# MoseleyBioinformaticsLab/pdb_eda

Measured on NVIDIA B200. Metric: voxels/s (atom-sphere voxels + blob-CCL voxels per pass of the voxel hot path), higher is better.
Workload: dtype f64

## Files before the change

### include/pdbeda_b200.h

```cpp
#ifndef PDBEDA_B200_H
#define PDBEDA_B200_H

#include <stdint.h>

#ifdef __cplusplus
extern "C" {
#endif

#define PE_ABI_VERSION 1

typedef enum pe_status {
    PE_OK = 0,
    PE_ERR_ARG = -1,
    PE_ERR_CUDA = -2,
    PE_ERR_CAPACITY = -3,
    PE_ERR_NO_DEVICE = -4
} pe_status;

typedef struct pe_geom {
    int32_t ncrs[3];
    int32_t crs_start[3];
    int32_t xyz_interval[3];
    int32_t crs_interval[3];
    int32_t unique_ncrs[3];
    int32_t map2xyz[3];
    int32_t map2crs[3];
    int32_t orthogonal;
    int32_t mv_perm[3];
    int32_t mv_fma;
    double grid_length[3];
    double origin[3];
    double ortho[9];
    double deortho[9];
} pe_geom;

int pe_abi_version(void);
const char *pe_last_error(void);
int pe_device_info(int32_t *sm_count, int32_t *cc_major, int32_t *cc_minor);

long long pe_launch_count(void);
void pe_profile_enable(int on);
void pe_profile_reset(void);
int pe_profile_entries(void);
int pe_profile_get(int index, const char **name, long long *count, double *total_ms);

int64_t pe_stats_workspace_bytes(void);
int pe_map_mean_std(const float *d_rho, int64_t n, double *d_out, void *d_ws, void *stream);
int pe_map_sum_abs(const float *d_rho, int64_t n, float cutoff, double *d_out, void *d_ws, void *stream);
int pe_sum_abs_f64(const double *d_values, int64_t n, float cutoff, double *d_out, void *d_ws, void *stream);

int pe_point_density(const pe_geom *g, const float *d_rho, int64_t n, const int32_t *d_crs, float *d_rho_out,
                     uint8_t *d_valid, void *stream);
int pe_xyz2crs(const pe_geom *g, int64_t n, const double *d_xyz, int32_t *d_crs, void *stream);
int pe_crs2xyz(const pe_geom *g, int64_t n, const int32_t *d_crs, double *d_xyz, void *stream);

#define PE_SPHERE_NOUT 8
int64_t pe_sphere_workspace_bytes(int64_t n_atoms);
int pe_sphere_union_warp_cycles(unsigned long long *out5);
int pe_sphere_sums(const pe_geom *g, const float *d_rho, int32_t n_atoms, const double *d_xyz,
                   const float *d_radius, int32_t n_groups, const int32_t *d_group_start, float cut_pos,
                   float cut_neg, double *d_out, void *d_ws, void *stream);
int pe_sphere_sums_atoms_and_groups(const pe_geom *g, const float *d_rho, int32_t n_atoms, const double *d_xyz,
                                    const float *d_atom_radius, float max_atom_radius, const float *d_group_radius,
                                    int32_t n_groups, const int32_t *d_group_start, float cut_pos, float cut_neg,
                                    double *d_out_atoms, double *d_out_groups, void *d_ws, void *stream);

typedef struct pe_sums_map {
    pe_geom geom;
    const float *d_rho;
    float cut_pos;
    float cut_neg;
} pe_sums_map;
int64_t pe_batch_sphere_sums_workspace_bytes(int64_t n_atoms);
int pe_batch_sphere_sums(int32_t n_maps, const pe_sums_map *d_maps, int32_t n_atoms, const double *d_xyz, const float *d_radius,
                         int32_t n_groups, const int32_t *d_group_map, const int32_t *d_group_start, const int32_t *d_atom_start,
                         double *d_out, void *d_ws, void *stream);

int pe_sphere_count(const pe_geom *g, const float *d_rho, int32_t n_atoms, const double *d_xyz,
                    const float *d_radius, float cutoff, int32_t *d_count, int32_t *d_box, void *stream);
int pe_sphere_fill(const pe_geom *g, const float *d_rho, int32_t n_atoms, const double *d_xyz,
                   const float *d_radius, float cutoff, const int64_t *d_offset, int32_t max_box_voxels,
                   int32_t *d_index, float *d_value, int32_t *d_label, void *stream);

int64_t pe_blob_workspace_bytes(const pe_geom *g, int64_t cap_voxels);
int pe_blob_stage_times(unsigned long long *out12);
int pe_blob_label(const pe_geom *g, const float *d_rho, float cut_pos, float cut_neg, int64_t cap_voxels,
                  int64_t cap_blobs, int64_t *d_counts, uint32_t *d_key, float *d_value, int32_t *d_label,
                  double *d_stats, void *d_ws, void *stream);

int64_t pe_slab_exchange_bytes(int64_t cap_blobs, int64_t cap_plane);
int64_t pe_slab_workspace_bytes(int32_t world, int64_t cap_blobs, int32_t u0, int32_t u1);
int pe_slab_boundary(const pe_geom *g_slab, int32_t u2_whole, int32_t s0, int32_t last_is_cut, const int64_t *d_counts,
                     int64_t cap_voxels, const uint32_t *d_key, const int32_t *d_label, int64_t cap_blobs, int64_t cap_plane,
                     void *d_exchange, void *d_ws, void *stream);
int pe_slab_merge(int32_t world, int32_t rank, const void *d_gathered, int64_t cap_blobs, int64_t cap_plane, int32_t u0,
                  int32_t u1, int32_t *d_new_number, int64_t *d_n_merged, void *d_ws, void *stream);
int pe_slab_relabel(const pe_geom *g_whole, int32_t u2_slab, int32_t s0, const int64_t *d_counts, int64_t cap_voxels,
                    const uint32_t *d_key, const float *d_value, int32_t *d_label, int64_t cap_blobs,
                    const int32_t *d_new_number, const int64_t *d_n_merged, int64_t cap_merged, double *d_stats, void *d_ws,
                    void *stream);
int pe_slab_status(const void *d_ws, void *stream, int32_t *bad);

int64_t pe_cluster_workspace_bytes(int64_t n);
int pe_cluster_crs(int64_t n, const int32_t *d_crs, int32_t *d_label, int64_t *d_nclusters, void *d_ws,
                   void *stream);
int pe_cluster_crs_grouped(int64_t n, const int32_t *d_crs, const int32_t *d_group, int32_t *d_label,
                           uint8_t *d_first, int64_t *d_nclusters, void *d_ws, void *stream);

int pe_crs_stats(const pe_geom *g, const float *d_rho, int64_t n, const int32_t *d_crs, const int32_t *d_label,
                 const uint8_t *d_take, int64_t n_clusters, double *d_stats, void *stream);

int pe_pair_metrics(const pe_geom *g, const float *d_rho_fo, const float *d_rho_diff, int64_t n, const int32_t *d_crs,
                    const int32_t *d_label, const uint8_t *d_take, int64_t n_groups, double *d_out, void *stream);

typedef struct pe_pair_map {
    pe_geom geom;
    const float *d_fo;
    const float *d_diff;
} pe_pair_map;
int64_t pe_pair_union_workspace_bytes(int32_t n_atoms);
int pe_pair_union_metrics(int32_t n_maps, const pe_pair_map *d_maps, int32_t n_groups, const int32_t *d_group_map,
                          const int32_t *d_group_start, const double *d_xyz, const float *d_radius, double *d_out, void *d_ws,
                          void *stream);

int64_t pe_overlap_workspace_bytes(int64_t n, int64_t cap_pairs);
int pe_overlap_pairs(int64_t n, const int32_t *d_crs, const int32_t *d_owner, const int32_t *d_group,
                     int64_t cap_pairs, int64_t *d_npairs, int32_t *d_pairs, void *d_ws, void *stream);
// ... 38 lines not shown
```

### pdb_eda_b200/_lib.py

```python
import ctypes
import os

_HERE = os.path.dirname(os.path.abspath(__file__))
LIB_PATH = os.path.join(_HERE, "csrc", "libpdbeda_b200.so")

PE_SPHERE_NOUT = 8


class PeGeom(ctypes.Structure):
    _fields_ = [
        ("ncrs", ctypes.c_int32 * 3),
        ("crs_start", ctypes.c_int32 * 3),
        ("xyz_interval", ctypes.c_int32 * 3),
        ("crs_interval", ctypes.c_int32 * 3),
        ("unique_ncrs", ctypes.c_int32 * 3),
        ("map2xyz", ctypes.c_int32 * 3),
        ("map2crs", ctypes.c_int32 * 3),
        ("orthogonal", ctypes.c_int32),
        ("mv_perm", ctypes.c_int32 * 3),
        ("mv_fma", ctypes.c_int32),
        ("grid_length", ctypes.c_double * 3),
        ("origin", ctypes.c_double * 3),
        ("ortho", ctypes.c_double * 9),
        ("deortho", ctypes.c_double * 9),
    ]


class PeBatchMap(ctypes.Structure):
    _fields_ = [("geom", PeGeom), ("d_rho", ctypes.c_void_p), ("cutoff", ctypes.c_float), ("atom_begin", ctypes.c_int32),
                ("atom_end", ctypes.c_int32), ("reserved", ctypes.c_int32)]


class PeSumsMap(ctypes.Structure):
    _fields_ = [("geom", PeGeom), ("d_rho", ctypes.c_void_p), ("cut_pos", ctypes.c_float), ("cut_neg", ctypes.c_float)]


class PePairMap(ctypes.Structure):
    _fields_ = [("geom", PeGeom), ("d_fo", ctypes.c_void_p), ("d_diff", ctypes.c_void_p)]


class PdbEdaLibError(RuntimeError):
    pass


_P = ctypes.c_void_p
_I32 = ctypes.c_int32
_I64 = ctypes.c_int64
_F32 = ctypes.c_float
_GEOM = ctypes.POINTER(PeGeom)

SIGNATURES = {
    "pe_abi_version": (ctypes.c_int, []),
    "pe_last_error": (ctypes.c_char_p, []),
    "pe_device_info": (ctypes.c_int, [ctypes.POINTER(_I32)] * 3),
    "pe_launch_count": (ctypes.c_longlong, []),
    "pe_profile_enable": (None, [ctypes.c_int]),
    "pe_profile_reset": (None, []),
    "pe_profile_entries": (ctypes.c_int, []),
    "pe_profile_get": (ctypes.c_int, [ctypes.c_int, ctypes.POINTER(ctypes.c_char_p), ctypes.POINTER(ctypes.c_longlong),
                                      ctypes.POINTER(ctypes.c_double)]),
    "pe_stats_workspace_bytes": (_I64, []),
    "pe_map_mean_std": (ctypes.c_int, [_P, _I64, _P, _P, _P]),
    "pe_map_sum_abs": (ctypes.c_int, [_P, _I64, _F32, _P, _P, _P]),
    "pe_sum_abs_f64": (ctypes.c_int, [_P, _I64, _F32, _P, _P, _P]),
    "pe_point_density": (ctypes.c_int, [_GEOM, _P, _I64, _P, _P, _P, _P]),
    "pe_xyz2crs": (ctypes.c_int, [_GEOM, _I64, _P, _P, _P]),
    "pe_crs2xyz": (ctypes.c_int, [_GEOM, _I64, _P, _P, _P]),
    "pe_sphere_workspace_bytes": (_I64, [_I64]),
    "pe_sphere_union_warp_cycles": (ctypes.c_int, [ctypes.POINTER(ctypes.c_ulonglong)]),
    "pe_sphere_sums": (ctypes.c_int, [_GEOM, _P, _I32, _P, _P, _I32, _P, _F32, _F32, _P, _P, _P]),
    "pe_sphere_sums_atoms_and_groups": (ctypes.c_int, [_GEOM, _P, _I32, _P, _P, _F32, _P, _I32, _P, _F32, _F32, _P, _P, _P, _P]),
    "pe_sphere_count": (ctypes.c_int, [_GEOM, _P, _I32, _P, _P, _F32, _P, _P, _P]),
    "pe_sphere_fill": (ctypes.c_int, [_GEOM, _P, _I32, _P, _P, _F32, _P, _I32, _P, _P, _P, _P]),
    "pe_blob_workspace_bytes": (_I64, [_GEOM, _I64]),
    "pe_blob_stage_times": (ctypes.c_int, [ctypes.POINTER(ctypes.c_ulonglong)]),
    "pe_blob_label": (ctypes.c_int, [_GEOM, _P, _F32, _F32, _I64, _I64, _P, _P, _P, _P, _P, _P, _P]),
    "pe_cluster_workspace_bytes": (_I64, [_I64]),
    "pe_cluster_crs": (ctypes.c_int, [_I64, _P, _P, _P, _P, _P]),
    "pe_cluster_crs_grouped": (ctypes.c_int, [_I64, _P, _P, _P, _P, _P, _P, _P]),
    "pe_crs_stats": (ctypes.c_int, [_GEOM, _P, _I64, _P, _P, _P, _I64, _P, _P]),
    "pe_pair_metrics": (ctypes.c_int, [_GEOM, _P, _P, _I64, _P, _P, _P, _I64, _P, _P]),
    "pe_batch_sphere_sums_workspace_bytes": (_I64, [_I64]),
    "pe_batch_sphere_sums": (ctypes.c_int, [_I32, _P, _I32, _P, _P, _I32, _P, _P, _P, _P, _P, _P]),
    "pe_pair_union_workspace_bytes": (_I64, [_I32]),
    "pe_pair_union_metrics": (ctypes.c_int, [_I32, _P, _I32, _P, _P, _P, _P, _P, _P, _P]),
    "pe_overlap_workspace_bytes": (_I64, [_I64, _I64]),
    "pe_overlap_pairs": (ctypes.c_int, [_I64, _P, _P, _P, _I64, _P, _P, _P, _P]),
    "pe_symmetry_workspace_bytes": (_I64, [_I32, _I32]),
    "pe_symmetry_expand": (ctypes.c_int, [_GEOM, _I32, _P, _I32, _P, _P, ctypes.POINTER(ctypes.c_double),
                                          ctypes.POINTER(ctypes.c_double), _I64, _P, _P, _P, _P, _P, _P]),
    "pe_nearest_atom": (ctypes.c_int, [_I64, _P, _I64, _P, _P, _P, _P]),
    "pe_slab_exchange_bytes": (_I64, [_I64, _I64]),
    "pe_slab_workspace_bytes": (_I64, [_I32, _I64, _I32, _I32]),
    "pe_slab_boundary": (ctypes.c_int, [_GEOM, _I32, _I32, _I32, _P, _I64, _P, _P, _I64, _I64, _P, _P, _P]),
    "pe_slab_merge": (ctypes.c_int, [_I32, _I32, _P, _I64, _I64, _I32, _I32, _P, _P, _P, _P]),
    "pe_slab_relabel": (ctypes.c_int, [_GEOM, _I32, _I32, _P, _I64, _P, _P, _P, _I64, _P, _P, _I64, _P, _P, _P]),
    "pe_slab_status": (ctypes.c_int, [_P, _P, ctypes.POINTER(_I32)]),
    "pe_cloud_workspace_bytes": (_I64, [_I64, _I64, _I64, _I64]),
    "pe_cloud_count": (ctypes.c_int, [_I32, _P, _I32, _P, _P, _P, _P, _P, _P, _P, _P]),
    "pe_cloud_aggregate": (ctypes.c_int, [_I32, _P, _I32, _P, _P, _P, _P, _P, _P, _P, _I32, _P, _I64, _I32, ctypes.c_double, _P, _P, _P,
                                          _P, _P]),
    "pe_cloud_status": (ctypes.c_int, [_P, _P, ctypes.POINTER(_I32)]),
    "pe_cloud_statistics": (ctypes.c_int, [_I32, _P, _I32, _P, _P, _P, _P, _I32, _P, _P, _P, _P, _I32, _P, _P, ctypes.c_double, _P, _P,
                                           _P, _P]),
}

_lib = None


def load():
    global _lib
    if _lib is not None:
        return _lib
    if not os.path.isfile(LIB_PATH):
        raise PdbEdaLibError(
            "%s not found: build it with `python -c 'import __graft_entry__ as g; g.build()'` or "
            "`make -C pdb_eda_b200/csrc` (there is no CPU fallback)" % LIB_PATH)
    lib = ctypes.CDLL(LIB_PATH)
    for name, (restype, argtypes) in SIGNATURES.items():
        fn = getattr(lib, name)
        fn.restype = restype
        fn.argtypes = argtypes
    if lib.pe_abi_version() != 1:
        raise PdbEdaLibError("libpdbeda_b200.so ABI version %d, expected 1" % lib.pe_abi_version())
    _lib = lib
    return lib


def check(rc, what):
    if rc != 0:
        msg = load().pe_last_error()
        raise PdbEdaLibError("%s failed (%d): %s" % (what, rc, msg.decode("utf-8", "replace") if msg else "?"))


def require_device():
    lib = load()
    sm, major, minor = _I32(0), _I32(0), _I32(0)
    check(lib.pe_device_info(ctypes.byref(sm), ctypes.byref(major), ctypes.byref(minor)), "pe_device_info")
    return sm.value, major.value, minor.value


def profile(enable=None, reset=False):
    lib = load()
# ... 16 lines not shown
```

### pdb_eda_b200/csrc/pe_blob.cu

```cuda
#include <cooperative_groups.h>
#include "pe_common.cuh"

namespace cg = cooperative_groups;

namespace pe {

constexpr int kBmpTx = 32;
constexpr int kBmpTy = 8;
constexpr int kSparseThreads = 512;
constexpr int kSegShift = 9;
constexpr int kSegWords = 1 << kSegShift;
constexpr int kChunkShift = 9;
constexpr int kChunkSmem = 4096;
constexpr int kScanBlocksPerSm = 2;
constexpr int kQueueCap = 160;
constexpr int kPoolWords = (kSparseThreads / 32) * 3 * kQueueCap > kChunkSmem ? (kSparseThreads / 32) * 3 * kQueueCap : kChunkSmem;
static_assert((1 << kChunkShift) == kSparseThreads, "a ranking chunk is one block of voxels");

struct BlobPlan {
    int U0, U1, U2, W;
    int64_t nwords;
    int64_t nwords_pad;
    int64_t nseg;
    int64_t cap;
// ... 573 lines not shown
}

}

using namespace pe;

extern "C" {

int pe_blob_stage_times(unsigned long long *out12) {
    PE_CHECK_ARG(out12 != nullptr, "pe_blob_stage_times: null pointer");
    PE_CUDA(cudaMemcpyFromSymbol(out12, g_stage_ns, sizeof(unsigned long long) * 12));
    return PE_OK;
}

int64_t pe_blob_workspace_bytes(const pe_geom *g, int64_t cap_voxels) {
    if (!g || cap_voxels < 0) return -1;
    return make_plan(g, cap_voxels).total;
}

int pe_blob_label(const pe_geom *g, const float *d_rho, float cut_pos, float cut_neg, int64_t cap_voxels,
                  int64_t cap_blobs, int64_t *d_counts, uint32_t *d_key, float *d_value, int32_t *d_label,
                  double *d_stats, void *d_ws, void *stream) {
    if (int rc = check_geom(g)) return rc;
    PE_CHECK_ARG(d_rho && d_counts && d_key && d_value && d_label && d_stats && d_ws, "pe_blob_label: null pointer");
    PE_CHECK_ARG(cap_voxels > 0 && cap_blobs > 0, "pe_blob_label: capacities must be positive");
    PE_CHECK_ARG(cap_voxels < (1ll << 30), "pe_blob_label: cap_voxels must be below 2^30");
    PE_CHECK_ARG(!(cut_pos < 0.f) && !(cut_neg > 0.f), "pe_blob_label: cut_pos must be >= 0 and cut_neg <= 0");
    PE_CHECK_ARG(cut_pos == cut_pos && cut_neg == cut_neg, "pe_blob_label: NaN cutoff");
    const BlobPlan p = make_plan(g, cap_voxels);
    PE_CHECK_ARG((int64_t)p.U0 * p.U1 * p.U2 < (1ll << 32), "pe_blob_label: unique volume too large for 32-bit keys");
    PE_CHECK_ARG(p.nwords_pad < (1ll << 31), "pe_blob_label: bit planes too large");
    cudaStream_t st = (cudaStream_t)stream;
    char *ws = (char *)d_ws;
    const int NC = g->ncrs[0], NR = g->ncrs[1];
    uint32_t *bmp = (uint32_t *)(ws + p.off_bmp);
    const bool use_pos = cut_pos > 0.f, use_neg = cut_neg < 0.f;

    PE_CUDA(cudaMemsetAsync(d_counts, 0, 5 * sizeof(int64_t), st));
    uint32_t *segcount = (uint32_t *)(ws + p.off_seg);
    PE_CUDA(cudaMemsetAsync(segcount, 0, (size_t)align_up(p.nseg * 4, 256) + 1024, st));
    {
        const bool vec4 = (NC % 4 == 0) && (((uintptr_t)d_rho & 15u) == 0);
        const int vec = vec4 ? 4 : 1;
        const int tx = kBmpTx, ty = kBmpTy;
        dim3 block(tx, ty, 1);
        dim3 grid(p.W / kWordsPerThread, (p.U0 + tx * vec - 1) / (tx * vec), (p.U1 + ty - 1) / ty);
        PE_CHECK_ARG(grid.y <= 65535 && grid.z <= 65535, "pe_blob_label: map too large for the launch grid");
        if (vec4)
            PE_LAUNCH("threshold_bitmap_kernel", st, threshold_bitmap_kernel<4><<<grid, block, 0, st>>>(
                d_rho, NC, NR, p.U0, p.U1, p.U2, p.W, cut_pos, cut_neg, use_pos, use_neg, bmp, bmp + p.nwords_pad, p.nwords_pad, segcount));
        else
            PE_LAUNCH("threshold_bitmap_kernel", st, threshold_bitmap_kernel<1><<<grid, block, 0, st>>>(
                d_rho, NC, NR, p.U0, p.U1, p.U2, p.W, cut_pos, cut_neg, use_pos, use_neg, bmp, bmp + p.nwords_pad, p.nwords_pad, segcount));
        PE_LAUNCH_CHECK();
    }
    SparseArgs a;
    a.rho = d_rho;
    a.NC = NC;
    a.NR = NR;
    a.U1 = p.U1;
    a.U2 = p.U2;
    a.W = p.W;
    a.nwords_pad = p.nwords_pad;
    a.cap = p.cap;
    a.cap_blobs = cap_blobs;
    a.nseg = (int)p.nseg;
    a.bmp = bmp;
    a.segcount = segcount;
    a.base = (uint32_t *)(ws + p.off_base);
    a.parent = (uint32_t *)(ws + p.off_parent);
    a.flags = (uint2 *)(ws + p.off_flags);
    a.coarse = (uint32_t *)(ws + p.off_coarse);
    a.nchunk_cap = p.nchunk_cap;
    a.counts = d_counts;
    a.key = d_key;
    a.value = d_value;
    a.label = d_label;
    a.stats = d_stats;
    static int blocks_per_sm = 0;
    if (blocks_per_sm == 0) {
        PE_CUDA(cudaOccupancyMaxActiveBlocksPerMultiprocessor(&blocks_per_sm, blob_sparse_kernel, kSparseThreads, 0));
        PE_CHECK_ARG(blocks_per_sm > 0, "pe_blob_label: the sparse kernel does not fit an SM");
    }
    const int nblocks = sm_count() * (blocks_per_sm < 3 ? blocks_per_sm : 3);
    a.p1_per_sm = blocks_per_sm == 3 ? kScanBlocksPerSm : (blocks_per_sm < 3 ? blocks_per_sm : 3);
    a.p1_blocks = sm_count() * a.p1_per_sm;
    a.sm_rank = (int *)(ws + p.off_seg + align_up(p.nseg * 4, 256));
    pe_geom geom = *g;
    void *args[] = {(void *)&geom, (void *)&a};
    PE_LAUNCH("blob_sparse_kernel", st,
              PE_CUDA(cudaLaunchCooperativeKernel((const void *)blob_sparse_kernel, dim3(nblocks), dim3(kSparseThreads), args, 0, st)));
    PE_LAUNCH_CHECK();
    return PE_OK;
}

}
```

### pdb_eda_b200/csrc/pe_common.cuh

```cuda
#pragma once
#include <cuda_runtime.h>
#include <stdint.h>
#include <stdio.h>
#include "../../include/pdbeda_b200.h"

namespace pe {

void set_error(const char *fmt, ...);

#define PE_CHECK_ARG(cond, ...)          \
    do {                                 \
        if (!(cond)) {                   \
            pe::set_error(__VA_ARGS__);  \
            return PE_ERR_ARG;           \
        }                                \
    } while (0)

#define PE_CUDA(call)                                                                         \
    do {                                                                                      \
        cudaError_t err__ = (call);                                                           \
        if (err__ != cudaSuccess) {                                                           \
            pe::set_error("%s failed at %s:%d: %s", #call, __FILE__, __LINE__,                \
                          cudaGetErrorString(err__));                                         \
            return PE_ERR_CUDA;                                                               \
        }                                                                                     \
    } while (0)

#define PE_LAUNCH_CHECK()                                                                     \
    do {                                                                                      \
        cudaError_t err__ = cudaGetLastError();                                               \
        if (err__ != cudaSuccess) {                                                           \
            pe::set_error("kernel launch failed at %s:%d: %s", __FILE__, __LINE__,            \
                          cudaGetErrorString(err__));                                         \
            return PE_ERR_CUDA;                                                               \
        }                                                                                     \
    } while (0)

struct ProfScope {
    int slot;
    cudaStream_t stream;
    ProfScope(const char *tag, cudaStream_t st);
    ~ProfScope();
};
#define PE_LAUNCH(tag, stream, ...)                          \
    do {                                                     \
        pe::ProfScope prof_scope__(tag, (cudaStream_t)(stream)); \
        __VA_ARGS__;                                         \
    } while (0)

int sm_count();
int check_geom(const pe_geom *g);
int check_geom_shape(const pe_geom *g, int64_t *nvox_out);

static inline int64_t align_up(int64_t x, int64_t a) { return (x + a - 1) / a * a; }

constexpr int kWarp = 32;
constexpr unsigned kFull = 0xffffffffu;
constexpr int kInvalidOff = (int)0x80000000;

__device__ __forceinline__ int sel3(int a0, int a1, int a2, int i) { return i == 0 ? a0 : (i == 1 ? a1 : a2); }
__device__ __forceinline__ double sel3(double a0, double a1, double a2, int i) { return i == 0 ? a0 : (i == 1 ? a1 : a2); }

__device__ __forceinline__ int floordiv(int a, int b) {
    int q = a / b;
    if ((a % b != 0) && ((a < 0) != (b < 0))) --q;
    return q;
}

__device__ __forceinline__ int wrap_index(int k, int n, int interval) {
    if (k < 0 || k >= n) k -= floordiv(k, interval) * interval;
    if ((n <= k && k < interval) || k < 0) return -1;
    return k;
}

__device__ __forceinline__ double mv_row(const double *a, double x0, double x1, double x2, const pe_geom &g) {
    const int p0 = g.mv_perm[0], p1 = g.mv_perm[1], p2 = g.mv_perm[2];
    const double a0 = a[p0], a1 = a[p1], a2 = a[p2];
    const double y0 = sel3(x0, x1, x2, p0), y1 = sel3(x0, x1, x2, p1), y2 = sel3(x0, x1, x2, p2);
    double acc = __dmul_rn(a0, y0);
    if (g.mv_fma) {
        acc = __fma_rn(a1, y1, acc);
        acc = __fma_rn(a2, y2, acc);
    } else {
        acc = __dadd_rn(acc, __dmul_rn(a1, y1));
        acc = __dadd_rn(acc, __dmul_rn(a2, y2));
    }
    return acc;
}

__device__ __forceinline__ int round_quotient(double a, double b) {
    const double q = __dmul_rn(a, __drcp_rn(b));
    const double r = rint(q);
    const double d = fabs(__dsub_rn(q, r));
    if (d < 0.499999999 && fabs(q) < 1.0e6) return (int)r;
    return (int)rint(__ddiv_rn(a, b));
}

__device__ __forceinline__ void xyz2crs(const pe_geom &g, double x, double y, double z, int &c, int &r, int &s) {
    int p0, p1, p2;
    if (g.orthogonal) {
        p0 = round_quotient(__dsub_rn(x, g.origin[0]), g.grid_length[0]);
        p1 = round_quotient(__dsub_rn(y, g.origin[1]), g.grid_length[1]);
        p2 = round_quotient(__dsub_rn(z, g.origin[2]), g.grid_length[2]);
    } else {
        const double f0 = mv_row(g.deortho + 0, x, y, z, g);
        const double f1 = mv_row(g.deortho + 3, x, y, z, g);
        const double f2 = mv_row(g.deortho + 6, x, y, z, g);
        p0 = (int)rint(__dmul_rn(f0, (double)g.xyz_interval[0])) - g.crs_start[g.map2xyz[0]];
        p1 = (int)rint(__dmul_rn(f1, (double)g.xyz_interval[1])) - g.crs_start[g.map2xyz[1]];
        p2 = (int)rint(__dmul_rn(f2, (double)g.xyz_interval[2])) - g.crs_start[g.map2xyz[2]];
    }
    c = sel3(p0, p1, p2, g.map2crs[0]);
    r = sel3(p0, p1, p2, g.map2crs[1]);
    s = sel3(p0, p1, p2, g.map2crs[2]);
}

__device__ __forceinline__ void crs2xyz(const pe_geom &g, int c, int r, int s, double &x, double &y, double &z) {
    const int k0 = sel3(c, r, s, g.map2xyz[0]);
    const int k1 = sel3(c, r, s, g.map2xyz[1]);
    const int k2 = sel3(c, r, s, g.map2xyz[2]);
    if (g.orthogonal) {
        x = __dadd_rn(__dmul_rn((double)k0, g.grid_length[0]), g.origin[0]);
        y = __dadd_rn(__dmul_rn((double)k1, g.grid_length[1]), g.origin[1]);
        z = __dadd_rn(__dmul_rn((double)k2, g.grid_length[2]), g.origin[2]);
    } else {
        const double f0 = __ddiv_rn((double)(k0 + g.crs_start[g.map2xyz[0]]), (double)g.xyz_interval[0]);
        const double f1 = __ddiv_rn((double)(k1 + g.crs_start[g.map2xyz[1]]), (double)g.xyz_interval[1]);
        const double f2 = __ddiv_rn((double)(k2 + g.crs_start[g.map2xyz[2]]), (double)g.xyz_interval[2]);
        x = mv_row(g.ortho + 0, f0, f1, f2, g);
        y = mv_row(g.ortho + 3, f0, f1, f2, g);
        z = mv_row(g.ortho + 6, f0, f1, f2, g);
    }
}
// ... 119 lines not shown
```

### pdb_eda_b200/csrc/pe_union.cu

```cuda
#include <limits.h>
#include <stddef.h>
#include "pe_sphere_dev.cuh"

#ifndef PE_UNION_PHASE_CYCLES
#define PE_UNION_PHASE_CYCLES 0
#endif

namespace pe {

__device__ unsigned long long g_union_warp_cycles[5];
struct PhaseClock {
#if PE_UNION_PHASE_CYCLES
    long long mark, t[5];
    __device__ __forceinline__ static long long now() {
#ifdef __CUDA_ARCH__
        return clock64();
#else
        return 0;
#endif
    }
    __device__ __forceinline__ PhaseClock() : mark(now()), t{0, 0, 0, 0, 0} {}
    __device__ __forceinline__ void lap(int k) {
        const long long now = PhaseClock::now();
        t[k] += now - mark;
// ... 222 lines not shown
                                if (!(dist2(ax, ay, az, vx, vy, vz) <= T)) continue;
                                atomicOr(&w.bits[(r - tr0) * kUT + (s - ts0)], 1u << (c - tc0));
                            }
                            __syncwarp();
                        }
                    }
                    clk.lap(1);
                    if (checked) {
                        if (has_neg)
                            gather_tile<true, true>(w, rho, acc, cp, cn, lane, tR, tS);
                        else
                            gather_tile<true, false>(w, rho, acc, cp, cn, lane, tR, tS);
                    } else {
                        if (has_neg)
                            gather_tile<false, true>(w, rho, acc, cp, cn, lane, tR, tS);
                        else
                            gather_tile<false, false>(w, rho, acc, cp, cn, lane, tR, tS);
                    }
                    __syncwarp();
                    clk.lap(3);
                }
    }
    const int n_all = warp_sum(acc.n_all), n_pos = warp_sum(acc.n_pos), n_neg = warp_sum(acc.n_neg);
    const int bad = warp_sum(acc.bad);
    const double s_all = warp_sum(acc.s_all), s_pos = warp_sum(acc.s_pos), s_neg = warp_sum(acc.s_neg);
    if (lane == 0) {
        o[0] = (double)n_all;
        o[1] = s_all;
        o[2] = (double)n_pos;
        o[3] = s_pos;
        o[4] = (double)n_neg;
        o[5] = s_neg;
        o[6] = bad ? 0.0 : 1.0;
        o[7] = candidates;
    }
    clk.lap(4);
}

template <int MODE>
__global__ void __launch_bounds__(kUW * 32, kUCtas)
    sphere_union_warp_kernel(const __grid_constant__ pe_geom g, const float *__restrict__ rho, int n_groups,
                             const int32_t *__restrict__ group_start, const double *__restrict__ xyz, const float *__restrict__ radius,
                             int32_t *box, double *thr, float cp, float cn, int *__restrict__ counter,
                             double *__restrict__ out , int n_quad_atoms,
                             const float *__restrict__ atom_radius, double *__restrict__ out_atoms ) {
    __shared__ WarpUnion wsh[kUW];
    const int warp = threadIdx.x >> 5, lane = threadIdx.x & 31;
    WarpUnion &w = wsh[warp];
    cp = eff_pos(cp);
    cn = eff_neg(cn);
    const bool has_neg = cn > __int_as_float(0xff800000);
    const int icx = g.map2crs[0];
    const float inv_gl = (float)(1.0 / g.grid_length[icx]);
    for (int i = lane; i < kUT * kUT; i += 32) w.bits[i] = 0u;
    __syncwarp();
    PhaseClock clk;
    const int n_items = n_groups + (n_quad_atoms + kAtomsPerWarp - 1) / kAtomsPerWarp;
    for (;;) {
        int item = 0;
        if (lane == 0) item = atomicAdd(counter, 1);
        item = __shfl_sync(kFull, item, 0);
        if (item >= n_items) break;
        if (item >= n_groups) {
            const int a0 = (item - n_groups) * kAtomsPerWarp;
            if (!quad_sums<MODE>(g, rho, n_quad_atoms, a0, xyz, atom_radius, cp, cn, quad_tabs(w), lane, out_atoms) &&
                lane < min(kAtomsPerWarp, n_quad_atoms - a0) * PE_SPHERE_NOUT)
                out_atoms[(int64_t)a0 * PE_SPHERE_NOUT + lane] = __longlong_as_double(0x7ff8000000000000ll);
            continue;
        }
        const int grp = item;
        union_group<MODE>(w, g, rho, group_start[grp], group_start[grp + 1], xyz, radius, box, thr, cp, cn, has_neg, icx, inv_gl, lane,
                          out + (int64_t)grp * PE_SPHERE_NOUT, clk);
    }
    clk.flush(lane);
}

int launch_union_warp(const pe_geom *g, const float *d_rho, int n_groups, const int32_t *d_group_start, const double *d_xyz,
                      const float *d_radius, int32_t *box, double *thr, float cut_pos, float cut_neg, int *d_counter, double *d_out,
                      int n_quad_atoms, const float *d_atom_radius, double *d_out_atoms, cudaStream_t st) {
    const int mode = z_axis_mode(g);
    PE_CUDA(cudaMemsetAsync(d_counter, 0, sizeof(int), st));
    const int warps_needed = n_groups + (n_quad_atoms + kAtomsPerWarp - 1) / kAtomsPerWarp;
    int grid = (warps_needed + kUW - 1) / kUW;
    const int max_grid = sm_count() * kUCtas;
    if (grid > max_grid) grid = max_grid;
    if (mode == 0)
        PE_LAUNCH("sphere_union_kernel", st, sphere_union_warp_kernel<0><<<grid, kUW * 32, 0, st>>>(
            *g, d_rho, n_groups, d_group_start, d_xyz, d_radius, box, thr, cut_pos, cut_neg, d_counter, d_out,
            n_quad_atoms, d_atom_radius, d_out_atoms));
    else if (mode == 1)
        PE_LAUNCH("sphere_union_kernel", st, sphere_union_warp_kernel<1><<<grid, kUW * 32, 0, st>>>(
            *g, d_rho, n_groups, d_group_start, d_xyz, d_radius, box, thr, cut_pos, cut_neg, d_counter, d_out,
            n_quad_atoms, d_atom_radius, d_out_atoms));
    else
        PE_LAUNCH("sphere_union_kernel", st, sphere_union_warp_kernel<2><<<grid, kUW * 32, 0, st>>>(
            *g, d_rho, n_groups, d_group_start, d_xyz, d_radius, box, thr, cut_pos, cut_neg, d_counter, d_out,
            n_quad_atoms, d_atom_radius, d_out_atoms));
    PE_LAUNCH_CHECK();
    return PE_OK;
}

constexpr int kUBatchCtas = 6;
struct WarpUnionGeom {
    WarpUnion u;
    pe_geom geom;
};
static_assert(kUBatchCtas * (kUW * sizeof(WarpUnionGeom) + 1024) <= 228 * 1024, "kUBatchCtas CTAs per SM do not fit the shared memory");

__global__ void __launch_bounds__(kUW * 32, kUBatchCtas)
    batch_union_kernel(int n_maps, const pe_sums_map *__restrict__ maps, int n_groups, const int32_t *__restrict__ group_map,
                       const int32_t *__restrict__ group_start, const double *__restrict__ xyz, const float *__restrict__ radius,
                       int32_t *box, double *thr, int *__restrict__ counter, double *__restrict__ out ) {
    __shared__ WarpUnionGeom wsh[kUW];
    const int warp = threadIdx.x >> 5, lane = threadIdx.x & 31;
    WarpUnion &w = wsh[warp].u;
    for (int i = lane; i < kUT * kUT; i += 32) w.bits[i] = 0u;
    __syncwarp();
    PhaseClock clk;
    for (;;) {
        int item = 0;
        if (lane == 0) item = atomicAdd(counter, 1);
        item = __shfl_sync(kFull, item, 0);
        if (item >= n_groups) break;
        const int grp = item;
        double *o = out + (int64_t)grp * PE_SPHERE_NOUT;
        const int m = group_map[grp];
        const bool bad_map = m < 0 || m >= n_maps;
        float cp = bad_map ? 0.f : maps[m].cut_pos, cn = bad_map ? 0.f : maps[m].cut_neg;
        if (bad_map || cp < 0.f || cn > 0.f) {
            if (lane < PE_SPHERE_NOUT) o[lane] = __longlong_as_double(0x7ff8000000000000ll);
            continue;
        }
        static_assert(sizeof(pe_geom) % 4 == 0, "pe_geom is copied as 32-bit words");
        for (int i = lane; i < (int)(sizeof(pe_geom) / 4); i += 32)
            reinterpret_cast<int *>(&wsh[warp].geom)[i] = reinterpret_cast<const int *>(&maps[m].geom)[i];
        __syncwarp();
        const pe_geom &g = wsh[warp].geom;
        const float *rho = maps[m].d_rho;
        cp = eff_pos(cp);
        cn = eff_neg(cn);
        const bool has_neg = cn > __int_as_float(0xff800000);
        const int icx = g.map2crs[0];
        const float inv_gl = (float)(1.0 / g.grid_length[icx]);
        const int a0 = group_start[grp], a1 = group_start[grp + 1];
        const int mode = g.map2xyz[2] == 1 ? 0 : (g.map2xyz[2] == 2 ? 1 : 2);
        if (mode == 0)
            union_group<0>(w, g, rho, a0, a1, xyz, radius, box, thr, cp, cn, has_neg, icx, inv_gl, lane, o, clk);
        else if (mode == 1)
            union_group<1>(w, g, rho, a0, a1, xyz, radius, box, thr, cp, cn, has_neg, icx, inv_gl, lane, o, clk);
        else
            union_group<2>(w, g, rho, a0, a1, xyz, radius, box, thr, cp, cn, has_neg, icx, inv_gl, lane, o, clk);
        __syncwarp();
    }
    clk.flush(lane);
}

int launch_batch_union(int n_maps, const pe_sums_map *d_maps, int n_groups, const int32_t *d_group_map, const int32_t *d_group_start,
                       const double *d_xyz, const float *d_radius, int32_t *box, double *thr, int *d_counter, double *d_out,
                       cudaStream_t st) {
    PE_CUDA(cudaMemsetAsync(d_counter, 0, sizeof(int), st));
    int grid = (n_groups + kUW - 1) / kUW;
    const int max_grid = sm_count() * kUBatchCtas;
    if (grid > max_grid) grid = max_grid;
    PE_LAUNCH("batch_union_kernel", st, batch_union_kernel<<<grid, kUW * 32, 0, st>>>(
        n_maps, d_maps, n_groups, d_group_map, d_group_start, d_xyz, d_radius, box, thr, d_counter, d_out));
    PE_LAUNCH_CHECK();
    return PE_OK;
// ... 12 lines not shown
```

### pdb_eda_b200/pipeline.py

```python
import ctypes

import numpy as np
import torch

from . import _device
from ._device import _ptr, _stream
from ._lib import PE_SPHERE_NOUT, check


class VoxelPass:
    def __init__(self, densityDev, diffDev, xyz, radii, residueStart, regionRadius=3.5, densityCutoff=None,
                 diffCutoff=None, capVoxels=None, capBlobs=None):
        self.dens = densityDev
        self.diff = diffDev
        dev = densityDev.device
        self.device = dev
        self.lib = densityDev.lib
        self.xyz = _device._as_dev(xyz, torch.float64, dev, (-1, 3))
        self.n_atoms = self.xyz.shape[0]
        self.radii = _device._as_dev(radii, torch.float32, dev, (-1,))
        self.max_radius = float(self.radii.max().item()) if self.n_atoms else 0.0
        self.region_radii = torch.full((self.n_atoms,), float(np.float32(regionRadius)), dtype=torch.float32, device=dev)
        self.res_start = _device._as_dev(residueStart, torch.int32, dev, (-1,))
        self.n_res = self.res_start.numel() - 1
        if densityCutoff is None:
            m, s = densityDev.mean_std()
            densityCutoff = m + 1.5 * s
        if diffCutoff is None:
            m, s = diffDev.mean_std()
            diffCutoff = m + 3.0 * s
        self.density_cut = float(np.float32(densityCutoff))
        self.diff_cut = float(np.float32(diffCutoff))
        self.cloud_out = torch.empty((self.n_atoms, PE_SPHERE_NOUT), dtype=torch.float64, device=dev)
        self.region_out = torch.empty((self.n_res, PE_SPHERE_NOUT), dtype=torch.float64, device=dev)
        self.sphere_ws = torch.empty(max(int(self.lib.pe_sphere_workspace_bytes(self.n_atoms)), 256), dtype=torch.uint8, device=dev)
        g = diffDev.geom
        nvox = g.unique_ncrs[0] * g.unique_ncrs[1] * g.unique_ncrs[2]
        self.n_blob_voxels = nvox
        self.cap_voxels = int(capVoxels or max(4096, nvox // 64))
        self.cap_blobs = int(capBlobs or max(1024, self.cap_voxels // 4))
        self.blob_counts = torch.zeros(5, dtype=torch.int64, device=dev)
        self.blob_key = torch.empty(2 * self.cap_voxels, dtype=torch.int32, device=dev)
        self.blob_value = torch.empty(2 * self.cap_voxels, dtype=torch.float32, device=dev)
        self.blob_label = torch.empty(2 * self.cap_voxels, dtype=torch.int32, device=dev)
        self.blob_stats = torch.empty((2 * self.cap_blobs, 8), dtype=torch.float64, device=dev)
        self.blob_ws = torch.empty(max(int(self.lib.pe_blob_workspace_bytes(ctypes.byref(g), self.cap_voxels)), 256),
                                   dtype=torch.uint8, device=dev)

    def spheres(self):
        check(self.lib.pe_sphere_sums_atoms_and_groups(
            ctypes.byref(self.dens.geom), _ptr(self.dens.rho), self.n_atoms, _ptr(self.xyz), _ptr(self.radii),
            ctypes.c_float(self.max_radius), _ptr(self.region_radii), self.n_res, _ptr(self.res_start),
            ctypes.c_float(self.density_cut), ctypes.c_float(0.0), _ptr(self.cloud_out), _ptr(self.region_out),
            _ptr(self.sphere_ws), _stream()), "pe_sphere_sums_atoms_and_groups")

    def blobs(self):
        check(self.lib.pe_blob_label(ctypes.byref(self.diff.geom), _ptr(self.diff.rho), ctypes.c_float(self.diff_cut),
                                     ctypes.c_float(-self.diff_cut), self.cap_voxels, self.cap_blobs, _ptr(self.blob_counts),
                                     _ptr(self.blob_key), _ptr(self.blob_value), _ptr(self.blob_label), _ptr(self.blob_stats),
                                     _ptr(self.blob_ws), _stream()), "pe_blob_label")

    def step(self):
        if getattr(self, "_side", None) is None:
            self._side = torch.cuda.Stream(device=self.device)
            self._fork, self._join = torch.cuda.Event(), torch.cuda.Event()
        main = torch.cuda.current_stream()
        self._fork.record(main)
        self._side.wait_event(self._fork)
        with torch.cuda.stream(self._side):
            self.blobs()
        self.spheres()
        self._join.record(self._side)
        main.wait_event(self._join)

    def stepFromHost(self, hostDensity, hostDiff, hostXyz=None):
        if getattr(self, "_copy", None) is None:
            self._copy = torch.cuda.Stream(device=self.device)
            self._ev = [torch.cuda.Event() for _ in range(3)]
        ev_free, ev_dens, ev_diff = self._ev
        main = torch.cuda.current_stream()
        ev_free.record(main)
        self._copy.wait_event(ev_free)
        with torch.cuda.stream(self._copy):
            self.dens.rho.copy_(hostDensity.view(-1), non_blocking=True)
            if hostXyz is not None:
                self.xyz.copy_(hostXyz, non_blocking=True)
            ev_dens.record(self._copy)
            self.diff.rho.copy_(hostDiff.view(-1), non_blocking=True)
            ev_diff.record(self._copy)
        main.wait_event(ev_dens)
        self.spheres()
        main.wait_event(ev_diff)
        self.blobs()
        return self.results()

    def _host_buffers(self):
        if getattr(self, "_h", None) is None:
            pin = lambda t: torch.empty(t.shape, dtype=t.dtype).pin_memory()
            self._h = {"cloud": pin(self.cloud_out), "region": pin(self.region_out), "counts": pin(self.blob_counts),
                       "key": pin(self.blob_key), "label": pin(self.blob_label), "stats": pin(self.blob_stats)}
        return self._h

    def results(self):
        h = self._host_buffers()
        h["cloud"].copy_(self.cloud_out, non_blocking=True)
        h["region"].copy_(self.region_out, non_blocking=True)
        h["counts"].copy_(self.blob_counts, non_blocking=True)
        torch.cuda.current_stream().synchronize()
        counts = h["counts"].numpy().copy()
        if counts[4]:
            raise RuntimeError("blob capacities too small: %s voxels / %s blobs needed" % (max(counts[0], counts[2]), max(counts[1], counts[3])))
        spans = []
        for k in range(2):
            nfg, nb = int(counts[2 * k]), int(counts[2 * k + 1])
            v0, b0 = k * self.cap_voxels, k * self.cap_blobs
            h["key"][v0:v0 + nfg].copy_(self.blob_key[v0:v0 + nfg], non_blocking=True)
            h["label"][v0:v0 + nfg].copy_(self.blob_label[v0:v0 + nfg], non_blocking=True)
            h["stats"][b0:b0 + nb].copy_(self.blob_stats[b0:b0 + nb], non_blocking=True)
            spans.append((v0, nfg, b0, nb))
        torch.cuda.current_stream().synchronize()
        out = {"cloud": h["cloud"].numpy(), "region": h["region"].numpy(), "blob_counts": counts}
        for (v0, nfg, b0, nb), tag in zip(spans, ("green", "red")):
            out[tag] = {"key": h["key"].numpy()[v0:v0 + nfg], "label": h["label"].numpy()[v0:v0 + nfg], "stats": h["stats"].numpy()[b0:b0 + nb]}
        return out

    def unit_counts(self):
        cloud = float(self.cloud_out[:, 0].sum().item())
        region = float(self.region_out[:, 0].sum().item())
        return cloud, region, float(self.n_blob_voxels)
```

Before: 485.6 billion.

## Run blob and sphere passes on disjoint SM partitions via green contexts

Adds CUDA green-context SM partitioning, so the blob CCL pass runs on 48 SMs and the sphere union kernel runs on the remaining SMs, each on its own stream. Grid sizes are now taken from the SM count of the launching stream. The aim is to stop the two concurrent passes from contending for the same SMs and to get more predictable overlap. In exchange, each pass has fewer SMs, the split is fixed, and there is extra event synchronisation plus dependence on driver entry points.

```diff
diff --git a/include/pdbeda_b200.h b/include/pdbeda_b200.h
--- a/include/pdbeda_b200.h
+++ b/include/pdbeda_b200.h
@@ -43,6 +43,10 @@
 void pe_profile_reset(void);
 int pe_profile_entries(void);
 int pe_profile_get(int index, const char **name, long long *count, double *total_ms);
+
+int pe_sm_partition_create(int32_t device, int32_t blob_sms, void **stream_blob, void **stream_rest, int32_t *sms_blob,
+                           int32_t *sms_rest);
+int pe_sm_partition_destroy(void *stream_blob, void *stream_rest);
 
 int64_t pe_stats_workspace_bytes(void);
 int pe_map_mean_std(const float *d_rho, int64_t n, double *d_out, void *d_ws, void *stream);
diff --git a/pdb_eda_b200/_lib.py b/pdb_eda_b200/_lib.py
--- a/pdb_eda_b200/_lib.py
+++ b/pdb_eda_b200/_lib.py
@@ -59,6 +59,8 @@
     "pe_profile_entries": (ctypes.c_int, []),
     "pe_profile_get": (ctypes.c_int, [ctypes.c_int, ctypes.POINTER(ctypes.c_char_p), ctypes.POINTER(ctypes.c_longlong),
                                       ctypes.POINTER(ctypes.c_double)]),
+    "pe_sm_partition_create": (ctypes.c_int, [_I32, _I32, ctypes.POINTER(_P), ctypes.POINTER(_P), ctypes.POINTER(_I32), ctypes.POINTER(_I32)]),
+    "pe_sm_partition_destroy": (ctypes.c_int, [_P, _P]),
     "pe_stats_workspace_bytes": (_I64, []),
     "pe_map_mean_std": (ctypes.c_int, [_P, _I64, _P, _P, _P]),
     "pe_map_sum_abs": (ctypes.c_int, [_P, _I64, _F32, _P, _P, _P]),
diff --git a/pdb_eda_b200/csrc/pe_blob.cu b/pdb_eda_b200/csrc/pe_blob.cu
--- a/pdb_eda_b200/csrc/pe_blob.cu
+++ b/pdb_eda_b200/csrc/pe_blob.cu
@@ -679,9 +679,10 @@
         PE_CUDA(cudaOccupancyMaxActiveBlocksPerMultiprocessor(&blocks_per_sm, blob_sparse_kernel, kSparseThreads, 0));
         PE_CHECK_ARG(blocks_per_sm > 0, "pe_blob_label: the sparse kernel does not fit an SM");
     }
-    const int nblocks = sm_count() * (blocks_per_sm < 3 ? blocks_per_sm : 3);
+    const int sms = stream_sm_count(st);
+    const int nblocks = sms * (blocks_per_sm < 3 ? blocks_per_sm : 3);
     a.p1_per_sm = blocks_per_sm == 3 ? kScanBlocksPerSm : (blocks_per_sm < 3 ? blocks_per_sm : 3);
-    a.p1_blocks = sm_count() * a.p1_per_sm;
+    a.p1_blocks = sms * a.p1_per_sm;
     a.sm_rank = (int *)(ws + p.off_seg + align_up(p.nseg * 4, 256));
     pe_geom geom = *g;
     void *args[] = {(void *)&geom, (void *)&a};
diff --git a/pdb_eda_b200/csrc/pe_common.cuh b/pdb_eda_b200/csrc/pe_common.cuh
--- a/pdb_eda_b200/csrc/pe_common.cuh
+++ b/pdb_eda_b200/csrc/pe_common.cuh
@@ -49,6 +49,7 @@
     } while (0)
 
 int sm_count();
+int stream_sm_count(cudaStream_t st);
 int check_geom(const pe_geom *g);
 int check_geom_shape(const pe_geom *g, int64_t *nvox_out);
 
diff --git a/pdb_eda_b200/csrc/pe_partition.cu b/pdb_eda_b200/csrc/pe_partition.cu
--- /dev/null
+++ b/pdb_eda_b200/csrc/pe_partition.cu
@@ -0,0 +1,195 @@
+#include <cuda.h>
+#include <cudaTypedefs.h>
+#include <mutex>
+#include <utility>
+#include <vector>
+#include "pe_common.cuh"
+
+namespace pe {
+namespace {
+
+struct Driver {
+    PFN_cuDeviceGet_v2000 deviceGet = nullptr;
+    PFN_cuDeviceGetDevResource_v12040 deviceGetDevResource = nullptr;
+    PFN_cuDevSmResourceSplitByCount_v12040 smResourceSplitByCount = nullptr;
+    PFN_cuDevResourceGenerateDesc_v12040 resourceGenerateDesc = nullptr;
+    PFN_cuGreenCtxCreate_v12040 greenCtxCreate = nullptr;
+    PFN_cuGreenCtxDestroy_v12040 greenCtxDestroy = nullptr;
+    PFN_cuGreenCtxGetDevResource_v12040 greenCtxGetDevResource = nullptr;
+    PFN_cuGreenCtxStreamCreate_v12050 greenCtxStreamCreate = nullptr;
+    PFN_cuStreamGetGreenCtx_v12040 streamGetGreenCtx = nullptr;
+    PFN_cuStreamSynchronize_v2000 streamSynchronize = nullptr;
+    PFN_cuStreamDestroy_v4000 streamDestroy = nullptr;
+    bool ok = false;
+};
+
+template <class F>
+bool entry(const char *name, unsigned version, F &fn) {
+    void *p = nullptr;
+    cudaDriverEntryPointQueryResult q = cudaDriverEntryPointSymbolNotFound;
+    if (cudaGetDriverEntryPointByVersion(name, &p, version, cudaEnableDefault, &q) != cudaSuccess || q != cudaDriverEntryPointSuccess || !p) {
+        cudaGetLastError();
+        return false;
+    }
+    fn = reinterpret_cast<F>(p);
+    return true;
+}
+
+const Driver *driver() {
+    static Driver d;
+    static std::once_flag once;
+    std::call_once(once, [] {
+        d.ok = entry("cuDeviceGet", 2000, d.deviceGet) && entry("cuDeviceGetDevResource", 12040, d.deviceGetDevResource) &&
+               entry("cuDevSmResourceSplitByCount", 12040, d.smResourceSplitByCount) &&
+               entry("cuDevResourceGenerateDesc", 12040, d.resourceGenerateDesc) && entry("cuGreenCtxCreate", 12040, d.greenCtxCreate) &&
+               entry("cuGreenCtxDestroy", 12040, d.greenCtxDestroy) && entry("cuGreenCtxGetDevResource", 12040, d.greenCtxGetDevResource) &&
+               entry("cuGreenCtxStreamCreate", 12050, d.greenCtxStreamCreate) && entry("cuStreamGetGreenCtx", 12040, d.streamGetGreenCtx) &&
+               entry("cuStreamSynchronize", 2000, d.streamSynchronize) && entry("cuStreamDestroy", 4000, d.streamDestroy);
+    });
+    return d.ok ? &d : nullptr;
+}
+
+struct Partition {
+    CUgreenCtx ctx[2] = {nullptr, nullptr};
+    CUstream stream[2] = {nullptr, nullptr};
+};
+
+std::mutex g_mutex;
+std::vector<Partition> g_partitions;
+std::vector<std::pair<cudaStream_t, int>> g_stream_sms;
+
+int release(const Driver *d, Partition &p, bool report) {
+    int rc = PE_OK;
+    for (int i = 0; i < 2; ++i) {
+        if (p.stream[i]) {
+            const CUresult s = d->streamSynchronize(p.stream[i]);
+            const CUresult r = d->streamDestroy(p.stream[i]);
+            if (s != CUDA_SUCCESS || r != CUDA_SUCCESS) {
+                if (report && rc == PE_OK) set_error("pe_sm_partition_destroy: stream %d: cuStreamSynchronize %d, cuStreamDestroy %d", i, (int)s, (int)r);
+                rc = PE_ERR_CUDA;
+            }
+            p.stream[i] = nullptr;
+        }
+    }
+    for (int i = 0; i < 2; ++i) {
+        if (p.ctx[i]) {
+            const CUresult r = d->greenCtxDestroy(p.ctx[i]);
+            if (r != CUDA_SUCCESS) {
+                if (report && rc == PE_OK) set_error("pe_sm_partition_destroy: cuGreenCtxDestroy failed (%d)", (int)r);
+                rc = PE_ERR_CUDA;
+            }
+            p.ctx[i] = nullptr;
+        }
+    }
+    return rc;
+}
+
+#define PE_DRV(call)                                                                   \
+    do {                                                                               \
+        const CUresult r__ = (call);                                                   \
+        if (r__ != CUDA_SUCCESS) {                                                     \
+            pe::set_error("pe_sm_partition_create: %s failed (CUresult %d)", #call, (int)r__); \
+            return PE_ERR_CUDA;                                                        \
+        }                                                                              \
+    } while (0)
+
+int create(const Driver *d, int device, int blob_sms, Partition &p, int sms[2]) {
+    PE_CUDA(cudaInitDevice(device, 0, 0));
+    CUdevice dev = 0;
+    PE_DRV(d->deviceGet(&dev, device));
+    CUdevResource all{};
+    PE_DRV(d->deviceGetDevResource(dev, &all, CU_DEV_RESOURCE_TYPE_SM));
+    PE_CHECK_ARG(blob_sms < (int)all.sm.smCount, "pe_sm_partition_create: blob_sms %d leaves none of the device's %u SMs", blob_sms,
+                 all.sm.smCount);
+    CUdevResource res[2] = {};
+    unsigned groups = 1;
+    PE_DRV(d->smResourceSplitByCount(&res[0], &groups, &all, &res[1], 0, (unsigned)blob_sms));
+    PE_CHECK_ARG(groups == 1 && (int)res[0].sm.smCount == blob_sms && res[1].sm.smCount > 0,
+                 "pe_sm_partition_create: the driver splits %d SMs as %u group(s) of %u and %u left (device of %u SMs)", blob_sms, groups,
+                 groups ? res[0].sm.smCount : 0u, res[1].sm.smCount, all.sm.smCount);
+    for (int i = 0; i < 2; ++i) {
+        CUdevResourceDesc desc = nullptr;
+        PE_DRV(d->resourceGenerateDesc(&desc, &res[i], 1));
+        PE_DRV(d->greenCtxCreate(&p.ctx[i], desc, dev, CU_GREEN_CTX_DEFAULT_STREAM));
+        PE_DRV(d->greenCtxStreamCreate(&p.stream[i], p.ctx[i], CU_STREAM_NON_BLOCKING, 0));
+        CUdevResource got{};
+        PE_DRV(d->greenCtxGetDevResource(p.ctx[i], &got, CU_DEV_RESOURCE_TYPE_SM));
+        sms[i] = (int)got.sm.smCount;
+    }
+    return PE_OK;
+}
+
+}
+
+int stream_sm_count(cudaStream_t st) {
+    std::lock_guard<std::mutex> lock(g_mutex);
+    for (const auto &e : g_stream_sms)
+        if (e.first == st) return e.second;
+    int n = sm_count();
+    if (const Driver *d = driver()) {
+        CUgreenCtx g = nullptr;
+        CUdevResource r{};
+        if (d->streamGetGreenCtx((CUstream)st, &g) == CUDA_SUCCESS && g &&
+            d->greenCtxGetDevResource(g, &r, CU_DEV_RESOURCE_TYPE_SM) == CUDA_SUCCESS && r.sm.smCount > 0)
+            n = (int)r.sm.smCount;
+    }
+    if (g_stream_sms.size() >= 64) g_stream_sms.clear();
+    g_stream_sms.emplace_back(st, n);
+    return n;
+}
+
+}
+
+extern "C" {
+
+int pe_sm_partition_create(int32_t device, int32_t blob_sms, void **stream_blob, void **stream_rest, int32_t *sms_blob,
+                           int32_t *sms_rest) {
+    PE_CHECK_ARG(stream_blob && stream_rest && sms_blob && sms_rest, "pe_sm_partition_create: null pointer");
+    *stream_blob = *stream_rest = nullptr;
+    *sms_blob = *sms_rest = 0;
+    PE_CHECK_ARG(blob_sms > 0, "pe_sm_partition_create: blob_sms must be positive (got %d)", blob_sms);
+    int ndev = 0;
+    if (cudaGetDeviceCount(&ndev) != cudaSuccess || ndev == 0) {
+        cudaGetLastError();
+        pe::set_error("no CUDA device is visible");
+        return PE_ERR_NO_DEVICE;
+    }
+    PE_CHECK_ARG(device >= 0 && device < ndev, "pe_sm_partition_create: device %d of %d", device, ndev);
+    const pe::Driver *d = pe::driver();
+    if (!d) {
+        pe::set_error("pe_sm_partition_create: the CUDA driver has no green-context entry points");
+        return PE_ERR_CUDA;
+    }
+    std::lock_guard<std::mutex> lock(pe::g_mutex);
+    pe::Partition p;
+    int sms[2] = {0, 0};
+    const int rc = pe::create(d, device, blob_sms, p, sms);
+    if (rc != PE_OK) {
+        pe::release(d, p, false);
+        return rc;
+    }
+    pe::g_partitions.push_back(p);
+    pe::g_stream_sms.clear();
+    *stream_blob = (void *)p.stream[0];
+    *stream_rest = (void *)p.stream[1];
+    *sms_blob = sms[0];
+    *sms_rest = sms[1];
+    return PE_OK;
+}
+
+int pe_sm_partition_destroy(void *stream_blob, void *stream_rest) {
+    std::lock_guard<std::mutex> lock(pe::g_mutex);
+    for (size_t i = 0; i < pe::g_partitions.size(); ++i) {
+        pe::Partition &p = pe::g_partitions[i];
+        if ((void *)p.stream[0] == stream_blob && (void *)p.stream[1] == stream_rest) {
+            const int rc = pe::release(pe::driver(), p, true);
+            pe::g_partitions.erase(pe::g_partitions.begin() + i);
+            pe::g_stream_sms.clear();
+            return rc;
+        }
+    }
+    pe::set_error("pe_sm_partition_destroy: the streams are not a live partition of this library");
+    return PE_ERR_ARG;
+}
+
+}
diff --git a/pdb_eda_b200/csrc/pe_union.cu b/pdb_eda_b200/csrc/pe_union.cu
--- a/pdb_eda_b200/csrc/pe_union.cu
+++ b/pdb_eda_b200/csrc/pe_union.cu
@@ -328,7 +328,7 @@
     PE_CUDA(cudaMemsetAsync(d_counter, 0, sizeof(int), st));
     const int warps_needed = n_groups + (n_quad_atoms + kAtomsPerWarp - 1) / kAtomsPerWarp;
     int grid = (warps_needed + kUW - 1) / kUW;
-    const int max_grid = sm_count() * kUCtas;
+    const int max_grid = stream_sm_count(st) * kUCtas;
     if (grid > max_grid) grid = max_grid;
     if (mode == 0)
         PE_LAUNCH("sphere_union_kernel", st, sphere_union_warp_kernel<0><<<grid, kUW * 32, 0, st>>>(
diff --git a/pdb_eda_b200/pipeline.py b/pdb_eda_b200/pipeline.py
--- a/pdb_eda_b200/pipeline.py
+++ b/pdb_eda_b200/pipeline.py
@@ -1,11 +1,57 @@
+import atexit
 import ctypes
+import os
+import warnings
 
 import numpy as np
 import torch
 
-from . import _device
+from . import _device, _lib
 from ._device import _ptr, _stream
 from ._lib import PE_SPHERE_NOUT, check
+
+BLOB_SMS = 48
+_partitions = {}
+
+
+def blobSms():
+    text = os.environ.get("PDB_EDA_B200_BLOB_SMS")
+    if text is None:
+        return BLOB_SMS
+    try:
+        return int(text)
+    except ValueError:
+        return -1
+
+
+def smPartition(device, blobSms):
+    index = device.index if device.index is not None else torch.cuda.current_device()
+    key = (index, blobSms)
+    if key in _partitions:
+        return _partitions[key]
+    part = None
+    if blobSms != 0:
+        lib = _lib.load()
+        sb, sr, nb, nr = ctypes.c_void_p(), ctypes.c_void_p(), ctypes.c_int32(), ctypes.c_int32()
+        rc = lib.pe_sm_partition_create(index, blobSms, ctypes.byref(sb), ctypes.byref(sr), ctypes.byref(nb), ctypes.byref(nr))
+        if rc == 0:
+            dev = torch.device("cuda", index)
+            part = (torch.cuda.ExternalStream(sb.value, device=dev), torch.cuda.ExternalStream(sr.value, device=dev))
+        else:
+            warnings.warn("VoxelPass.step: no partition of %d SMs for the blob pass on cuda:%d (%s); the blob and sphere passes "
+                          "share the SMs" % (blobSms, index, lib.pe_last_error().decode("utf-8", "replace")), RuntimeWarning, stacklevel=3)
+    _partitions[key] = part
+    return part
+
+
+@atexit.register
+def releasePartitions():
+    lib = _lib.load() if _partitions else None
+    for key in list(_partitions):
+        part = _partitions.pop(key)
+        if part is not None:
+            check(lib.pe_sm_partition_destroy(ctypes.c_void_p(part[0].cuda_stream), ctypes.c_void_p(part[1].cuda_stream)),
+                  "pe_sm_partition_destroy")
 
 
 class VoxelPass:
@@ -61,16 +107,25 @@
                                      _ptr(self.blob_ws), _stream()), "pe_blob_label")
 
     def step(self):
+        part = smPartition(self.device, blobSms())
         if getattr(self, "_side", None) is None:
             self._side = torch.cuda.Stream(device=self.device)
-            self._fork, self._join = torch.cuda.Event(), torch.cuda.Event()
+            self._fork, self._join, self._join_rest = torch.cuda.Event(), torch.cuda.Event(), torch.cuda.Event()
         main = torch.cuda.current_stream()
         self._fork.record(main)
-        self._side.wait_event(self._fork)
-        with torch.cuda.stream(self._side):
+        blob_stream = part[0] if part is not None else self._side
+        blob_stream.wait_event(self._fork)
+        with torch.cuda.stream(blob_stream):
             self.blobs()
-        self.spheres()
-        self._join.record(self._side)
+        if part is not None:
+            part[1].wait_event(self._fork)
+            with torch.cuda.stream(part[1]):
+                self.spheres()
+            self._join_rest.record(part[1])
+            main.wait_event(self._join_rest)
+        else:
+            self.spheres()
+        self._join.record(blob_stream)
         main.wait_event(self._join)
 
     def stepFromHost(self, hostDensity, hostDiff, hostXyz=None):
diff --git a/profiles/c2_partition.py b/profiles/c2_partition.py
--- /dev/null
+++ b/profiles/c2_partition.py
@@ -0,0 +1,145 @@
+#!/usr/bin/env python3
+import argparse
+import json
+import os
+import subprocess
+import sys
+import time
+
+import numpy as np
+import torch
+
+ROOT = os.path.dirname(os.path.dirname(os.path.abspath(__file__)))
+sys.path.insert(0, ROOT)
+import bench
+from pdb_eda_b200 import _device, _lib, ccp4, pipeline, synthetic
+
+KS = (0, 16, 24, 32, 40, 48, 56)
+
+
+def card():
+    try:
+        out = subprocess.run(["nvidia-smi", "-i", "0", "--query-gpu=name,power.limit,clocks.max.sm", "--format=csv,noheader"],
+                             capture_output=True, text=True, timeout=30).stdout.strip()
+    except Exception as exc:
+        out = "nvidia-smi unavailable (%s)" % exc
+    return "%s; nvidia-smi: %s" % (torch.cuda.get_device_name(0), out)
+
+
+def build_pass():
+    work = bench.build_workload(bench.FULL, seed=2)
+    n, cell = work["n"], work["cell"]
+    geom = _device.geom_from_header(ccp4.DensityHeader.fromFileHeader(synthetic.ccp4Header((n, n, n), cell, (n, n, n))))
+    dens = _device.DeviceMap(geom, torch.from_numpy(work["fofc2"].reshape(-1)).cuda())
+    diff = _device.DeviceMap(geom, torch.from_numpy(work["fofc"].reshape(-1)).cuda())
+    return pipeline.VoxelPass(dens, diff, work["xyz"].astype(np.float64), work["radii"], work["res_start"], bench.REGION_RADIUS)
+
+
+def per_step_ms(fn, steps, stream, warmup=20):
+    e0, e1 = torch.cuda.Event(enable_timing=True), torch.cuda.Event(enable_timing=True)
+    with torch.cuda.stream(stream):
+        for _ in range(warmup):
+            fn()
+        e0.record(stream)
+        for _ in range(steps):
+            fn()
+        e1.record(stream)
+    torch.cuda.synchronize()
+    return e0.elapsed_time(e1) / steps
+
+
+def compare(a, b):
+    bad = [k for k in ("cloud", "region", "blob_counts") if not np.array_equal(a[k], b[k])]
+    bad += ["%s %s" % (t, k) for t in ("green", "red") for k in ("key", "label") if not np.array_equal(a[t][k], b[t][k])]
+    if bad:
+        return "DIFFERENT: " + ", ".join(bad)
+    rel = 0.0
+    for t in ("green", "red"):
+        x, y = a[t]["stats"], b[t]["stats"]
+        if not np.array_equal(x, y):
+            rel = max(rel, float(np.max(np.abs(x - y) / np.maximum(np.abs(y), 1e-300))))
+    return "identical" if rel == 0.0 else "sums within %.1e relative" % rel
+
+
+def snapshot(res):
+    return {k: (v.copy() if isinstance(v, np.ndarray) else {kk: vv.copy() for kk, vv in v.items()}) for k, v in res.items()}
+
+
+def main():
+    ap = argparse.ArgumentParser()
+    ap.add_argument("--out", default=None, help="markdown report (default: stdout only)")
+    ap.add_argument("--steps", type=int, default=2000)
+    ap.add_argument("--repeats", type=int, default=3)
+    ap.add_argument("--profile-steps", type=int, default=300)
+    ap.add_argument("--alone-steps", type=int, default=1000)
+    args = ap.parse_args()
+    _device.require_cuda()
+    torch.cuda.set_device(0)
+    t0 = time.time()
+    vp = build_pass()
+    setup_s = time.time() - t0
+    main_stream = torch.cuda.current_stream()
+    sms_total = _lib.require_device()[0]
+    results, same = {}, {}
+    for k in KS:
+        os.environ["PDB_EDA_B200_BLOB_SMS"] = str(k)
+        vp.step()
+        results[k] = snapshot(vp.results())
+        assert k == 0 or pipeline.smPartition(vp.device, k) is not None, "no partition of %d SMs" % k
+        same[k] = compare(results[k], results[0])
+
+    step_ms = {k: [] for k in KS}
+    for r in range(args.repeats):
+        order = KS[r % len(KS):] + KS[:r % len(KS)]
+        for k in order:
+            os.environ["PDB_EDA_B200_BLOB_SMS"] = str(k)
+            step_ms[k].append(per_step_ms(vp.step, args.steps, main_stream))
+
+    kernels = {}
+    for k in KS:
+        os.environ["PDB_EDA_B200_BLOB_SMS"] = str(k)
+        per_step_ms(vp.step, 20, main_stream)
+        _lib.profile(True, reset=True)
+        prof_ms = per_step_ms(vp.step, args.profile_steps, main_stream, warmup=0)
+        prof = _lib.profile()
+        _lib.profile(False)
+        kernels[k] = {"ms_per_step_profiled": prof_ms,
+                      "us_per_launch": {name: ms * 1e3 / max(c, 1) for name, (c, ms) in prof.items()}}
+
+    alone = {}
+    for k in KS:
+        part = pipeline.smPartition(vp.device, k) if k else None
+        bs, rs = (part[0], part[1]) if part else (main_stream, main_stream)
+        alone[k] = {"blobs_ms": per_step_ms(vp.blobs, args.alone_steps, bs), "spheres_ms": per_step_ms(vp.spheres, args.alone_steps, rs)}
+    os.environ.pop("PDB_EDA_B200_BLOB_SMS")
+
+    result = {"card": card(), "sms": sms_total, "steps": args.steps, "repeats": args.repeats, "setup_s": round(setup_s, 1),
+              "step_ms": step_ms, "kernels": kernels, "alone": alone, "results_vs_k0": same}
+    print(json.dumps(result))
+    lines = ["# C2 step on SM partitions (blob pass on k SMs, sphere kernel on the other %d - k)" % sms_total, "",
+             "Measured by `profiles/c2_partition.py` on %s." % result["card"], "",
+             "C2 workload of bench.py (384^3 map pair, %d atoms / %d residues, seed 2). ms/step by CUDA events over %d steps per "
+             "setting, settings alternated in %d rounds; k = 0 is the shared-SM two-stream schedule. Blob / sphere alone: that path "
+             "by itself on its partition's stream (%d calls)." % (vp.n_atoms, vp.n_res, args.steps, args.repeats, args.alone_steps), "",
+             "| k | ms/step (rounds) | median | blobs alone ms | spheres alone ms | max(alone) | threshold us | sparse us | sphere us | results vs k = 0 |",
+             "|---:|---|---:|---:|---:|---:|---:|---:|---:|---|"]
+    for k in KS:
+        u = kernels[k]["us_per_launch"]
+        lines.append("| %d | %s | %.4f | %.4f | %.4f | %.4f | %.1f | %.1f | %.1f | %s |" % (
+            k, " / ".join("%.4f" % x for x in step_ms[k]), float(np.median(step_ms[k])), alone[k]["blobs_ms"], alone[k]["spheres_ms"],
+            max(alone[k].values()), u.get("threshold_bitmap_kernel", float("nan")), u.get("blob_sparse_kernel", float("nan")),
+            u.get("sphere_union_kernel", float("nan")), same[k]))
+    lines += ["", "Per-kernel times are event pairs on each kernel's own stream in a profiled run; with two paths in flight they "
+              "include the time a kernel shares the GPU with the other path.", ""]
+    text = "\n".join(lines)
+    print(text)
+    if args.out:
+        os.makedirs(os.path.dirname(os.path.abspath(args.out)), exist_ok=True)
+        with open(args.out, "w") as f:
+            f.write(text)
+        with open(os.path.splitext(args.out)[0] + ".json", "w") as f:
+            json.dump(result, f, indent=1)
+
+
+if __name__ == "__main__":
+    main()
```

Result: faster. 588.8 billion (median of 6 runs) (+21.3%).
